# serviceberry3/weiner_slamit_v2

Hardware: AMD Instinct MI355X
Metric: frames/sec ORB extract+match @640x480x8lvl (higher is better)
Workload: dtype u8; 1 GPU; BASELINE configs[1]: 640x480 8-level ORB extract (1000 features, FAST 20/7) + brute-force 256-bit Hamming best/second match vs the stream's previous frame; 256 independent streams per GPU per step; distinct_frame_pairs_per_gpu=16, parallelism=streams sharded over 1 GPU(s), no data-path collective

## Files before the change

### weiner_slamit_v2_amd/csrc/orb_api.hip

```cpp
#include <hip/hip_runtime.h>
#include <math.h>
#include <stdio.h>
#include <stdlib.h>
#include <string.h>

#include <algorithm>
#include <vector>

#include "../../include/slamit.h"
#include "orb_plan.h"
#include "slamit_internal.h"

hipError_t orbk_upload_pattern(hipStream_t st);
void orbk_resize(hipStream_t st, const uint8_t* src, int sw, int sh, size_t sstride, size_t sframe,
                 uint8_t* dst, int dw, int dh, size_t dstride, size_t dframe, const int* xofs,
                 const short* ialpha, const int* yofs, const short* ibeta, int nframes);
void orbk_resize_rows4(hipStream_t st, const uint8_t* src, size_t sstride, size_t sframe, int sh, uint8_t* dst, int dw, int dh,
                       size_t dstride, size_t dframe, const uint32_t* d_col, const uint32_t* d_row, int nframes);
void orbk_resize_rows8(hipStream_t st, const uint8_t* src, size_t sstride, size_t sframe, int sh, uint8_t* dst, int dw, int dh,
                       size_t dstride, size_t dframe, const uint32_t* d_col8, const uint32_t* d_row, int nframes);
hipError_t orbk_pyramid_bands_prepare(int smem_bytes);
void orbk_pyramid_bands(hipStream_t st, const BandTab& tab, const uint8_t* d_tables, const BandRows* d_rows, int first, int last, int nbands,
                        const uint8_t* src, size_t sstride, size_t sframe, int sh, uint8_t* pyr, size_t pyr_frame, int tile0, int smem, int nframes);
hipError_t orbk_pyramid_prepare(int smem_bytes);
void orbk_pyramid(hipStream_t st, const OrbLevel* levels, int nlevels, const PyrBox* boxes, const PyrTabs* tabs,
                  int nregions, const uint8_t* img0, size_t img0_stride, size_t img0_frame, uint8_t* pyr, int bufA_bytes,
                  int smem_bytes, int nframes, int l_first, int l_last);
hipError_t orbk_fast_prepare(int max_wcell, int max_hcell);
void orbk_fast(hipStream_t st, const FastTab& tab, int nlevels, const uint32_t* d_cells, int cells_per_frame, const uint8_t* img0,
               size_t img0_stride, size_t img0_frame, const uint8_t* pyr, unsigned long long* cand,
               size_t cand_frame_stride, int* cand_count, int iniTh, int minTh, int max_wcell, int max_hcell, int nframes);
hipError_t orbk_octree_prepare(int node_cap, int key_cap);
void orbk_octree(hipStream_t st, const OrbLevel* levels, int nlevels, const unsigned long long* cand,
                 size_t cand_frame_stride, int* cand_count, uint32_t* ws_xy, uint16_t* ws_node,
                 OrbLevelKp* lkp, size_t kp_frame_stride, int* kp_count, int node_cap, int key_cap, int nframes,
                 int level_override);
void orbk_ic_angle(hipStream_t st, const OrbLevel* levels, int nlevels, const uint8_t* img0, size_t img0_stride,
                   size_t img0_frame, const uint8_t* pyr, OrbLevelKp* lkp, size_t kp_frame_stride,
                   const int* kp_count, int max_kp, int nframes);
void orbk_blur_stream(hipStream_t st, const OrbLevel* levels, const uint32_t* d_tiles, int ntiles, const uint8_t* img0,
                      size_t img0_stride, size_t img0_frame, const uint8_t* pyr, uint8_t* blur, int nframes, bool edge);
void orbk_blur(hipStream_t st, const OrbLevel* levels, const uint32_t* d_tiles, int total_tiles, const uint8_t* img0,
               size_t img0_stride, size_t img0_frame, const uint8_t* pyr, uint8_t* blur, int nframes);
void orbk_describe(hipStream_t st, const OrbLevel* levels, int nlevels, const uint8_t* blur,
                   const OrbLevelKp* lkp, size_t kp_frame_stride, const int* kp_count, slamit_kp* out_kps,
                   uint8_t* out_desc, int out_cap, int* out_n, int max_kp, int nframes);
void orbk_pad(hipStream_t st, const uint8_t* src, int w, int h, size_t sstride, uint8_t* dst);
void orbk_decode_candidates(hipStream_t st, const OrbLevel* levels, int level, const unsigned long long* K, int n,
                            unsigned long long* order_out, int* xys);

namespace {

inline size_t round_up(size_t v, size_t a) { return (v + a - 1) / a * a; }

}

#define ORB_BLUR_SPLIT 1

struct slamit_orb {
    slamit_orb_params p;
    int device;
    hipStream_t stream;
    hipStream_t stream_b;
    hipEvent_t ev_pyr, ev_mid, ev_blur;
    SlamitSwitches sw;
    int nlevels;
    OrbPlan pl;
    bool blur_stream_on;
    uint8_t* d_tables;
    const OrbLevel* d_levels;
    uint8_t* d_pyr;
    uint8_t* d_blur;
    unsigned long long* d_cand;
    uint32_t* d_ws_xy;
    uint16_t* d_ws_node;
    int* d_counts;
    bool counters_clean;
    OrbLevelKp* d_lkp;
    uint8_t* d_in;
    size_t d_in_stride, d_in_frame;
    slamit_kp* d_out_kps;
    uint8_t* d_out_desc;
    int* d_out_n;
    uint8_t* h_out;
    uint8_t* d_scratch;
    size_t scratch_bytes;
    int prof_on;
    long prof_call;
    std::vector<hipEvent_t> prof_ev;
    std::vector<int> prof_stage;
    const uint8_t* last_img0;
    size_t last_stride, last_frame;
    int last_nframes;
};

template <typename T>
static const T* dtab(const slamit_orb* h, size_t off) { return reinterpret_cast<const T*>(h->d_tables + off); }

static void orb_free(slamit_orb* h) {
    if (!h) return;
    SlamitDeviceGuard guard(h->device);
    hipFree(h->d_tables); hipFree(h->d_pyr); hipFree(h->d_blur); hipFree(h->d_cand); hipFree(h->d_ws_xy);
    hipFree(h->d_ws_node); hipFree(h->d_counts); hipFree(h->d_lkp); hipFree(h->d_in); hipFree(h->d_out_kps);
    hipFree(h->d_out_desc); hipFree(h->d_out_n); if (h->h_out) hipHostFree(h->h_out); hipFree(h->d_scratch);
    for (hipEvent_t e : h->prof_ev) hipEventDestroy(e);
    if (h->ev_pyr) hipEventDestroy(h->ev_pyr);
    if (h->ev_mid) hipEventDestroy(h->ev_mid);
    if (h->ev_blur) hipEventDestroy(h->ev_blur);
    if (h->stream_b) hipStreamDestroy(h->stream_b);
    if (h->stream) hipStreamDestroy(h->stream);
    delete h;
}

extern "C" {

int slamit_orb_create(const slamit_orb_params* p, int device, slamit_orb** out) {
    if (!p || !out) return slamit_fail(SLAMIT_ERR_ARG, "slamit_orb_create: null argument");
    *out = nullptr;
    if (p->nlevels < 1 || p->nlevels > ORB_MAX_LEVELS || p->nfeatures < 1 || !(p->scale_factor > 1.f) ||
        p->ini_th_fast < 1 || p->ini_th_fast > 255 || p->min_th_fast < 1 || p->min_th_fast > 255 ||
        p->width < 0 || p->height < 0 || p->max_batch < 1)
        return slamit_fail(SLAMIT_ERR_ARG, "slamit_orb_create: parameter out of range");
    SLAMIT_USE_DEVICE(device);
    slamit_orb* h = new slamit_orb();
    h->p = *p;
    h->device = device;
    h->sw = slamit_read_switches();
    const int nl = h->nlevels = p->nlevels;
    const char* why = "";
// ... 118 lines not shown
        }
    };
    prof_mark(h, st, ST_RESIZE, true);
    const bool src0_aligned = ((((uintptr_t)d_gray) | stride | frame_stride) & 3) == 0;
    const bool side = h->prof_on != 1;
    const bool early_blur = side && ORB_BLUR_SPLIT < nl - 1;
    int early_done = -1;
    auto fork_early_blur = [&](int l) -> hipError_t {
        hipError_t e = hipEventRecord(h->ev_mid, st);
        if (e == hipSuccess) e = hipStreamWaitEvent(h->stream_b, h->ev_mid, 0);
        if (e != hipSuccess) return e;
        launch_blur(h->stream_b, 0, l + 1);
        early_done = l;
        return hipSuccess;
    };
    if (!P.bands.empty() && src0_aligned) {
        for (const OrbBandSeg& G : P.bands) {
            const OrbLevel& S = P.levels[G.first];
            orbk_pyramid_bands(st, P.band_tab, h->d_tables, dtab<BandRows>(h, G.rows_off), G.first, G.last, G.nbands,
                               G.first == 0 ? d_gray : h->d_pyr + S.plane_off, G.first == 0 ? stride : (size_t)S.stride,
                               G.first == 0 ? frame_stride : P.pyr_frame_total, S.h, h->d_pyr, P.pyr_frame_total, G.tile0, G.smem, nframes);
            if (early_blur && G.last < nl - 1 && early_done < 0) HIP_TRY(fork_early_blur(G.last));
        }
    } else if (P.rows4_ok && src0_aligned) {
        for (int l = 1; l < nl; ++l) {
            const OrbLevel& S = P.levels[l - 1];
            const OrbLevel& D = P.levels[l];
            const uint8_t* src = l == 1 ? d_gray : h->d_pyr + S.plane_off;
            const OrbResizeTabs& T = P.rs[l];
            if (!T.col8.empty())
                orbk_resize_rows8(st, src, l == 1 ? stride : (size_t)S.stride, l == 1 ? frame_stride : P.pyr_frame_total, S.h,
                                  h->d_pyr + D.plane_off, D.w, D.h, (size_t)D.stride, P.pyr_frame_total, dtab<uint32_t>(h, T.col8_off),
                                  dtab<uint32_t>(h, T.row4_off), nframes);
            else
                orbk_resize_rows4(st, src, l == 1 ? stride : (size_t)S.stride, l == 1 ? frame_stride : P.pyr_frame_total, S.h,
                                  h->d_pyr + D.plane_off, D.w, D.h, (size_t)D.stride, P.pyr_frame_total, dtab<uint32_t>(h, T.col4_off),
                                  dtab<uint32_t>(h, T.row4_off), nframes);
            if (early_blur && l == ORB_BLUR_SPLIT) HIP_TRY(fork_early_blur(l));
        }
    } else if (P.pyr_regions) {
        orbk_pyramid(st, h->d_levels, nl, dtab<PyrBox>(h, P.boxes_off), dtab<PyrTabs>(h, P.tabs_off), P.pyr_regions, d_gray, stride, frame_stride,
                     h->d_pyr, P.pyr_bufA, P.pyr_smem, nframes, 0, nl - 1);
    } else {
        for (int l = 1; l < nl; ++l) {
            const OrbLevel& S = P.levels[l - 1];
            const OrbLevel& D = P.levels[l];
            const uint8_t* src = l == 1 ? d_gray : h->d_pyr + S.plane_off;
            size_t sstride = l == 1 ? stride : (size_t)S.stride;
            size_t sframe = l == 1 ? frame_stride : P.pyr_frame_total;
            const OrbResizeTabs& T = P.rs[l];
            orbk_resize(st, src, S.w, S.h, sstride, sframe, h->d_pyr + D.plane_off, D.w, D.h, (size_t)D.stride,
                        P.pyr_frame_total, dtab<int>(h, T.xofs_off), dtab<short>(h, T.ialpha_off), dtab<int>(h, T.yofs_off),
                        dtab<short>(h, T.ibeta_off), nframes);
        }
    }
    prof_mark(h, st, ST_RESIZE, false);
    prof_mark(h, st, ST_FAST, true);
    orbk_fast(st, P.fast, nl, dtab<uint32_t>(h, P.cells_off), (int)(P.cells.size() / 4), d_gray, stride, frame_stride, h->d_pyr, h->d_cand,
              P.cand_frame_stride, cand_count, h->p.ini_th_fast, h->p.min_th_fast, P.max_wcell, P.max_hcell, nframes);
    prof_mark(h, st, ST_FAST, false);
    if (side) {
        HIP_TRY(hipEventRecord(h->ev_pyr, st));
        HIP_TRY(hipStreamWaitEvent(h->stream_b, h->ev_pyr, 0));
        launch_blur(h->stream_b, early_done + 1, nl);
        HIP_TRY(hipEventRecord(h->ev_blur, h->stream_b));
    }
    prof_mark(h, st, ST_OCTREE, true);
    orbk_octree(st, h->d_levels, nl, h->d_cand, P.cand_frame_stride, cand_count, h->d_ws_xy, h->d_ws_node, h->d_lkp,
                P.kp_frame_stride, kp_count, P.node_cap, P.oct_key_cap, nframes, -1);
    prof_mark(h, st, ST_OCTREE, false);
    prof_mark(h, st, ST_ANGLE, true);
    orbk_ic_angle(st, h->d_levels, nl, d_gray, stride, frame_stride, h->d_pyr, h->d_lkp, P.kp_frame_stride, kp_count,
                  P.max_kp_level, nframes);
    prof_mark(h, st, ST_ANGLE, false);
    if (side) {
        HIP_TRY(hipStreamWaitEvent(st, h->ev_blur, 0));
    } else {
        prof_mark(h, st, ST_BLUR, true);
        launch_blur(st, 0, nl);
        prof_mark(h, st, ST_BLUR, false);
    }
    prof_mark(h, st, ST_DESCRIBE, true);
    orbk_describe(st, h->d_levels, nl, h->d_blur, h->d_lkp, P.kp_frame_stride, kp_count, d_kps, d_desc, cap, d_n_out,
                  P.max_kp_level, nframes);
    prof_mark(h, st, ST_DESCRIBE, false);
    ++h->prof_call;
    HIP_TRY(hipGetLastError());
    h->counters_clean = true;
    h->last_img0 = d_gray; h->last_stride = stride; h->last_frame = frame_stride; h->last_nframes = nframes;
    return SLAMIT_OK;
}

int slamit_orb_extract_batch(slamit_orb* h, const uint8_t* gray, size_t stride, size_t frame_stride, int nframes,
                             slamit_kp* kps, uint8_t* desc, int cap, int* n_out) {
    if (!h || !n_out || nframes < 0) return slamit_fail(SLAMIT_ERR_ARG, "slamit_orb_extract_batch: bad argument");
    if (nframes > h->p.max_batch) return slamit_fail(SLAMIT_ERR_CAPACITY, "slamit_orb_extract_batch: nframes > max_batch");
    if (nframes == 0) return SLAMIT_OK;
    if (h->p.width == 0 || h->p.height == 0) {
        for (int f = 0; f < nframes; ++f) n_out[f] = 0;
        return SLAMIT_OK;
    }
    if (!gray || !kps || !desc) return slamit_fail(SLAMIT_ERR_ARG, "slamit_orb_extract_batch: null buffer");
    if (cap < h->pl.max_out) return slamit_fail(SLAMIT_ERR_CAPACITY, "slamit_orb_extract_batch: cap < slamit_orb_max_keypoints()");
    SLAMIT_USE_DEVICE(h->device);
    const int W = h->p.width, H = h->p.height;
    for (int f = 0; f < nframes; ++f)
        HIP_TRY(hipMemcpy2DAsync(h->d_in + f * h->d_in_frame, h->d_in_stride, gray + (size_t)f * frame_stride, stride, W, H,
                                 hipMemcpyHostToDevice, h->stream));
    int rc = slamit_orb_extract_batch_dev(h, h->d_in, h->d_in_stride, h->d_in_frame, nframes, h->d_out_kps, h->d_out_desc,
                                          h->pl.max_out, h->d_out_n, h->stream);
    if (rc != SLAMIT_OK) return rc;
    const size_t o_k = ((sizeof(int) * (size_t)nframes + 255) & ~(size_t)255), kb = sizeof(slamit_kp) * (size_t)h->pl.max_out * nframes;
    const size_t o_d = (o_k + kb + 255) & ~(size_t)255, db = (size_t)SLAMIT_DESC_BYTES * h->pl.max_out * nframes;
    HIP_TRY(hipMemcpyAsync(h->h_out, h->d_out_n, sizeof(int) * nframes, hipMemcpyDeviceToHost, h->stream));
    HIP_TRY(hipMemcpyAsync(h->h_out + o_k, h->d_out_kps, kb, hipMemcpyDeviceToHost, h->stream));
    HIP_TRY(hipMemcpyAsync(h->h_out + o_d, h->d_out_desc, db, hipMemcpyDeviceToHost, h->stream));
    HIP_TRY(hipStreamSynchronize(h->stream));
    memcpy(n_out, h->h_out, sizeof(int) * nframes);
    for (int f = 0; f < nframes; ++f) {
        const int n = n_out[f];
        if (n > 0) {
            memcpy(kps + (size_t)f * cap, h->h_out + o_k + sizeof(slamit_kp) * (size_t)f * h->pl.max_out, sizeof(slamit_kp) * n);
            memcpy(desc + (size_t)f * cap * SLAMIT_DESC_BYTES, h->h_out + o_d + (size_t)SLAMIT_DESC_BYTES * f * h->pl.max_out, (size_t)SLAMIT_DESC_BYTES * n);
        }
    }
    return SLAMIT_OK;
}

int slamit_orb_extract(slamit_orb* h, const uint8_t* gray, size_t stride, slamit_kp* kps, uint8_t* desc, int cap,
                       int* n_out) {
    return slamit_orb_extract_batch(h, gray, stride, stride * (size_t)(h ? h->p.height : 0), 1, kps, desc, cap, n_out);
}

int slamit_orb_profile(slamit_orb* h, int enable, float* stage_ms, int32_t* stage_calls, int nstages) {
    if (!h) return slamit_fail(SLAMIT_ERR_ARG, "slamit_orb_profile: null handle");
    SLAMIT_USE_DEVICE(h->device);
    if (stage_ms || stage_calls) {
        for (int i = 0; i < nstages; ++i) { if (stage_ms) stage_ms[i] = 0.f; if (stage_calls) stage_calls[i] = 0; }
        for (size_t i = 0; i < h->prof_stage.size() && 2 * i + 1 < h->prof_ev.size(); ++i) {
            HIP_TRY(hipEventSynchronize(h->prof_ev[2 * i + 1]));
            float ms = 0.f;
            HIP_TRY(hipEventElapsedTime(&ms, h->prof_ev[2 * i], h->prof_ev[2 * i + 1]));
            int s = h->prof_stage[i];
            if (s < nstages) { if (stage_ms) stage_ms[s] += ms; if (stage_calls) stage_calls[s] += 1; }
        }
    }
    for (hipEvent_t e : h->prof_ev) hipEventDestroy(e);
    h->prof_ev.clear(); h->prof_stage.clear();
    h->prof_on = enable;
    h->prof_call = 0;
    return SLAMIT_OK;
}

int slamit_orb_level(slamit_orb* h, int frame, int level, uint8_t* dst, size_t dst_bytes, int* w, int* h_out) {
    if (!h || level < 0 || level >= h->nlevels) return slamit_fail(SLAMIT_ERR_ARG, "slamit_orb_level: bad level");
    if (h->p.width == 0 || h->p.height == 0) return slamit_fail(SLAMIT_ERR_STATE, "slamit_orb_level: empty image");
    const OrbLevel& L = h->pl.levels[level];
    if (w) *w = L.w;
    if (h_out) *h_out = L.h;
    if (!dst) return SLAMIT_OK;
    if (frame < 0 || frame >= h->last_nframes || !h->last_img0) return slamit_fail(SLAMIT_ERR_STATE, "slamit_orb_level: no such frame in the last extract call");
    size_t need = (size_t)(L.w + 38) * (L.h + 38);
    if (dst_bytes < need) return slamit_fail(SLAMIT_ERR_CAPACITY, "slamit_orb_level: dst too small");
    SLAMIT_USE_DEVICE(h->device);
    const uint8_t* src = level == 0 ? h->last_img0 + (size_t)frame * h->last_frame
                                    : h->d_pyr + L.plane_off + (size_t)frame * h->pl.pyr_frame_total;
    orbk_pad(h->stream, src, L.w, L.h, level == 0 ? h->last_stride : (size_t)L.stride, h->d_scratch);
// ... 68 lines not shown
```

### weiner_slamit_v2_amd/csrc/orb_kernels.hip

```cpp
#include <hip/hip_runtime.h>
#include <stdint.h>

#include <algorithm>

#include "orb_types.h"
#include "slamit_math.h"
#include "wave_ops.h"
#include "../../include/slamit.h"
#include "../../include/slamit_orb_pattern.h"

#define WAVE 64

__global__ __launch_bounds__(256) void resize_level_kernel(
    const uint8_t* __restrict__ src, int sw, int sh, size_t sstride, size_t sframe,
    uint8_t* __restrict__ dst, int dw, int dh, size_t dstride, size_t dframe,
    const int* __restrict__ xofs, const short* __restrict__ ialpha,
    const int* __restrict__ yofs, const short* __restrict__ ibeta) {
    const int x4 = (blockIdx.x * 64 + (threadIdx.x & 63)) * 4;
    const int y = blockIdx.y * 4 + (threadIdx.x >> 6);
    const int f = blockIdx.z;
    if (x4 >= dw || y >= dh) return;
    const uint8_t* S = src + (size_t)f * sframe;
    int sy = yofs[y];
    int sy0 = min(max(sy, 0), sh - 1), sy1 = min(max(sy + 1, 0), sh - 1);
    const uint8_t* S0 = S + (size_t)sy0 * sstride;
    const uint8_t* S1 = S + (size_t)sy1 * sstride;
    int b0 = ibeta[2 * y], b1 = ibeta[2 * y + 1];
    uint32_t out = 0;
#pragma unroll
    for (int i = 0; i < 4; ++i) {
        int x = x4 + i;
        if (x < dw) {
            int sx = xofs[x];
            int sx1 = min(sx + 1, sw - 1);
            int a0 = ialpha[2 * x], a1 = ialpha[2 * x + 1];
            int r0 = S0[sx] * a0 + S0[sx1] * a1;
            int r1 = S1[sx] * a0 + S1[sx1] * a1;
            int v = ((((b0 * (r0 >> 4)) >> 16) + ((b1 * (r1 >> 4)) >> 16) + 2) >> 2) & 0xFF;
            out |= (uint32_t)v << (8 * i);
        }
    }
    *reinterpret_cast<uint32_t*>(dst + (size_t)f * dframe + (size_t)y * dstride + x4) = out;
}

typedef unsigned short rs_us2 __attribute__((ext_vector_type(2)));
typedef unsigned rs_u3 __attribute__((ext_vector_type(3)));
__device__ __forceinline__ uint32_t rs_dot2(uint32_t taps, uint32_t alpha) {
    return __builtin_amdgcn_udot2(__builtin_bit_cast(rs_us2, taps), __builtin_bit_cast(rs_us2, alpha), 0u, false);
}

#define RS_RP 2

template <int RP>
__device__ __forceinline__ void rs_item(const int item, const uint8_t* S, const unsigned ss, const unsigned sbytes, uint8_t* D, const unsigned dstride,
                                        const uint4* __restrict__ coltab, const uint2* __restrict__ rowtab, const int ngroups,
                                        const unsigned inv_groups, const int dh) {
    const int yq = (int)__umulhi((unsigned)item, inv_groups);
    const int g = item - yq * ngroups;
    const uint8_t* ct = reinterpret_cast<const uint8_t*>(coltab) + 48u * (unsigned)g;
    const uint4 c0 = *reinterpret_cast<const uint4*>(ct), c1 = *reinterpret_cast<const uint4*>(ct + 16u);
    const uint32_t c2x = *reinterpret_cast<const uint32_t*>(ct + 32u);
    int yrow[2 * RP];
    uint2 rt[2 * RP];
    {
        const uint4* rp4 = reinterpret_cast<const uint4*>(reinterpret_cast<const uint8_t*>(rowtab) + 16u * (unsigned)(RP * yq));
#pragma unroll
        for (int r = 0; r < RP; ++r) {
            const uint4 v = rp4[r];
            rt[2 * r] = make_uint2(v.x, v.y); rt[2 * r + 1] = make_uint2(v.z, v.w);
        }
#pragma unroll
        for (int r = 0; r < 2 * RP; ++r) yrow[r] = min(2 * RP * yq + r, dh - 1);
    }
    const unsigned b = c0.x & 0xFFFFu, sh = (c0.x >> 16) & 3u, off1 = (c0.x >> 20) & 15u, off2 = (c0.x >> 24) & 15u;
    const uint32_t sel[4] = {c0.y, c0.z, c0.w, c1.x}, al[4] = {c1.y, c1.z, c1.w, c2x};
    uint32_t w[4 * RP][3];
    const __amdgpu_buffer_rsrc_t rsrc = __builtin_amdgcn_make_buffer_rsrc(const_cast<uint8_t*>(S), 0, sbytes, 0x00020000);
    (void)off1; (void)off2;
#pragma unroll
    for (int r = 0; r < 4 * RP; ++r) {
        const unsigned srow = (r & 1) ? (rt[r >> 1].x >> 16) : (rt[r >> 1].x & 0xFFFFu);
        const unsigned ro = __umul24(srow, ss) + b;
        const rs_u3 v = __builtin_amdgcn_raw_buffer_load_b96(rsrc, (int)ro, 0, 0);
        w[r][0] = v.x; w[r][1] = v.y; w[r][2] = v.z;
    }
#pragma unroll
    for (int k = 0; k < 2 * RP; ++k) {
// ... 1419 lines not shown
    };
    auto rotate = [&]() {
        const blur_u3 ta = qa[0], tb = qb[0];
        qa[0] = qa[1]; qb[0] = qb[1]; qa[1] = qa[2]; qb[1] = qb[2]; qa[2] = ta; qb[2] = tb;
#pragma unroll
        for (int j = 0; j < 4; ++j) { P[0][j] = P[1][j]; P[1][j] = P[2][j]; P[2][j] = P[3][j]; }
    };
#define BLUR_OUT(f, k0, k1, k2, k3, j) \
    min((udot2(P[(f) & 3][j], k3, udot2(P[((f) + 3) & 3][j], k2, udot2(P[((f) + 2) & 3][j], k1, udot2(P[((f) + 1) & 3][j], k0, 1u << 15)))) >> 16), 255u)
#define BLUR_OUT_A(f) (BLUR_OUT(f, kA0, kA1, kA2, kA3, 0) | (BLUR_OUT(f, kA0, kA1, kA2, kA3, 1) << 8) | (BLUR_OUT(f, kA0, kA1, kA2, kA3, 2) << 16) | (BLUR_OUT(f, kA0, kA1, kA2, kA3, 3) << 24))
#define BLUR_OUT_B(f) (BLUR_OUT(f, kB0, kB1, kB2, kB3, 0) | (BLUR_OUT(f, kB0, kB1, kB2, kB3, 1) << 8) | (BLUR_OUT(f, kB0, kB1, kB2, kB3, 2) << 16) | (BLUR_OUT(f, kB0, kB1, kB2, kB3, 3) << 24))
    auto generic = [&](const int p) {
        const blur_u3 na = fetch(2 * p + 6), nb = fetch(2 * p + 7);
        advance(0, 3, na, nb);
        const int ya = 2 * p - 3, yb = 2 * p - 2;
        if (ya >= by0 && ya <= ylast) *reinterpret_cast<uint32_t*>(D + __umul24((unsigned)ya, ds)) = BLUR_OUT_A(3);
        if (yb >= by0 && yb <= ylast) *reinterpret_cast<uint32_t*>(D + __umul24((unsigned)yb, ds)) = BLUR_OUT_B(3);
        rotate();
    };
    int p = p0;
#pragma unroll
    for (int k = 0; k < 3; ++k, ++p) advance(k, k, fetch(2 * p + 6), fetch(2 * p + 7));
    generic(p);
    ++p;
    const int n = min((ylast + 2) >> 1, (h - 8) >> 1) - p + 1;
    int nu = 0;
    {
        const unsigned long long act = __ballot(1);
#pragma unroll
        for (int b = 32; b; b >>= 1) nu += __ballot(n >= nu + b) == act ? b : 0;
    }
    if (nu > 0) {
        const uint8_t* sp = S + __umul24((unsigned)(2 * p + 6), ss);
        uint8_t* dp = D + __umul24((unsigned)(2 * p - 3), ds);
        p += nu;
        auto steady = [&](const int q, const int f) {
            const blur_u3 na = fetch_row(sp);
            sp += ss;
            const blur_u3 nb = fetch_row(sp);
            sp += ss;
            advance(q, f, na, nb);
            *reinterpret_cast<uint32_t*>(dp) = BLUR_OUT_A(f);
            dp += ds;
            *reinterpret_cast<uint32_t*>(dp) = BLUR_OUT_B(f);
            dp += ds;
            asm volatile("" : "+v"(sp), "+v"(dp));
        };
        for (; nu >= 12; nu -= 12) {
#pragma unroll
            for (int u = 0; u < 12; ++u) {
                steady(u % 3, (u + 3) & 3);
                __builtin_amdgcn_sched_barrier(0);
            }
        }
        for (; nu >= 3; nu -= 3) {
#pragma unroll
            for (int u = 0; u < 3; ++u) {
                steady(u, (u + 3) & 3);
                __builtin_amdgcn_sched_barrier(0);
            }
#pragma unroll
            for (int j = 0; j < 4; ++j) { P[2][j] = P[1][j]; P[1][j] = P[0][j]; P[0][j] = P[3][j]; }
        }
#pragma unroll 1
        for (; nu > 0; --nu) {
            steady(0, 3);
            rotate();
        }
    }
#pragma unroll 4
    for (; p <= p1; ++p) generic(p);
#undef BLUR_OUT_B
#undef BLUR_OUT_A
#undef BLUR_OUT
}

__constant__ __attribute__((aligned(16))) signed char c_pattern[SLAMIT_ORB_PATTERN_INTS];
#define DESC_KP_PER_WAVE 4
#define DESC_R 18
#define DESC_ROWS (2 * DESC_R + 1)
#define DESC_PITCH 48
#define DESC_LOADS 2

__global__ __launch_bounds__(256) void describe_kernel(
    const OrbLevel* __restrict__ levels, int nlevels,
    const uint8_t* __restrict__ blur,
    const OrbLevelKp* __restrict__ lkp, size_t kp_frame_stride, const int* __restrict__ kp_count,
    slamit_kp* __restrict__ out_kps, uint8_t* __restrict__ out_desc, int out_cap,
    int* __restrict__ out_n, int xcd_frames , int kblocks) {
    const int lane = threadIdx.x & 63;
    int level, frame, kb;
    if (xcd_frames) {
        const unsigned w = blockIdx.x, k = w >> 3, P = (unsigned)(nlevels * kblocks), fq = k / P, local = k - fq * P;
        frame = (int)(8u * fq + ((w + fq) & 7u));
        if (frame >= xcd_frames) return;
        level = (int)(local / (unsigned)kblocks); kb = (int)(local - (unsigned)level * (unsigned)kblocks);
    } else { level = blockIdx.y; frame = blockIdx.z; kb = blockIdx.x; }
    const int i0 = (kb * 4 + (threadIdx.x >> 6)) * DESC_KP_PER_WAVE;
    const OrbLevel& L = levels[level];
    const int* counts = kp_count + frame * nlevels;
    int offset = 0, total = 0;
    for (int l = 0; l < nlevels; ++l) {
        int c = counts[l];
        if (l < level) offset += c;
        total += c;
    }
    if (level == 0 && i0 == 0 && lane == 0) out_n[frame] = min(total, out_cap);
    const int count = counts[level];
    if (i0 >= count) return;
    const int4 pw = reinterpret_cast<const int4*>(c_pattern)[lane];
    const int pt[4] = {pw.x, pw.y, pw.z, pw.w};
    float px0[4], py0[4], px1[4], py1[4];
#pragma unroll
    for (int t = 0; t < 4; ++t) {
        px0[t] = (float)(signed char)(pt[t] & 0xFF); py0[t] = (float)(signed char)((pt[t] >> 8) & 0xFF);
        px1[t] = (float)(signed char)((pt[t] >> 16) & 0xFF); py1[t] = (float)(signed char)((pt[t] >> 24) & 0xFF);
    }
    const uint8_t* img = blur + L.blur_off + (size_t)frame * L.blur_bytes;
    const unsigned step = (unsigned)L.stride;
    const OrbLevelKp* KP = lkp + L.kp_off + (size_t)frame * kp_frame_stride;
    OrbLevelKp kp[DESC_KP_PER_WAVE];
#pragma unroll
    for (int k = 0; k < DESC_KP_PER_WAVE; ++k) kp[k] = KP[min(i0 + k, count - 1)];
    __shared__ __attribute__((aligned(16))) uint8_t s_patch[4][DESC_KP_PER_WAVE][DESC_ROWS * DESC_PITCH];
    const int wv = threadIdx.x >> 6;
    int lrow[DESC_LOADS], lcol[DESC_LOADS];
    unsigned poff[DESC_LOADS];
#pragma unroll
    for (int it = 0; it < DESC_LOADS; ++it) {
        const int idx = lane + 64 * it;
        lrow[it] = (int)(((unsigned)idx * 21846u) >> 16);
        lcol[it] = idx - 3 * lrow[it];
        poff[it] = __umul24((unsigned)min(lrow[it], DESC_ROWS - 1), step) + 16u * (unsigned)lcol[it];
    }
    const __amdgpu_buffer_rsrc_t rsrc = __builtin_amdgcn_make_buffer_rsrc(const_cast<uint8_t*>(img), 0, (unsigned)L.stride * (unsigned)L.h, 0x00020000);
    typedef unsigned desc_u4 __attribute__((ext_vector_type(4)));
    desc_u4 ld[DESC_KP_PER_WAVE][DESC_LOADS];
#pragma unroll
    for (int k = 0; k < DESC_KP_PER_WAVE; ++k) {
        const unsigned base = __umul24((unsigned)(kp[k].y - DESC_R), step) + (unsigned)((kp[k].x - DESC_R) & ~3);
#pragma unroll
        for (int it = 0; it < DESC_LOADS; ++it) ld[k][it] = __builtin_amdgcn_raw_buffer_load_b128(rsrc, (int)(base + poff[it]), 0, 0);
    }
#pragma unroll
    for (int k = 0; k < DESC_KP_PER_WAVE; ++k)
#pragma unroll
        for (int it = 0; it < DESC_LOADS; ++it)
            if (lrow[it] < DESC_ROWS) *reinterpret_cast<desc_u4*>(&s_patch[wv][k][__mul24(lrow[it], DESC_PITCH) + 16 * lcol[it]]) = ld[k][it];
    __builtin_amdgcn_fence(__ATOMIC_ACQ_REL, "wavefront");
    __builtin_amdgcn_wave_barrier();
    typedef float desc_f2 __attribute__((ext_vector_type(2)));
    const desc_f2 magic = {12582912.0f, 12582912.0f};
    const unsigned DESC_BIAS = 0x400000u * (unsigned)DESC_PITCH + 0x4B400000u;
    int tv0[DESC_KP_PER_WAVE][4], tv1[DESC_KP_PER_WAVE][4];
#pragma unroll
    for (int k = 0; k < DESC_KP_PER_WAVE; ++k) {
        const float a = kp[k].cs, b = kp[k].sn;
        const desc_f2 ba = {b, a}, anb = {a, -b};
        const uint8_t* center = &s_patch[wv][k][DESC_R * DESC_PITCH + DESC_R + ((kp[k].x - DESC_R) & 3)];
        const uint8_t* biased = center - DESC_BIAS;
#pragma unroll
        for (int t = 0; t < 4; ++t) {
            const desc_f2 p0 = {px0[t], px0[t]}, q0 = {py0[t], py0[t]}, p1 = {px1[t], px1[t]}, q1 = {py1[t], py1[t]};
            const desc_f2 m0 = (p0 * ba + q0 * anb) + magic, m1 = (p1 * ba + q1 * anb) + magic;
            tv0[k][t] = biased[__umul24(__float_as_uint(m0.x), (unsigned)DESC_PITCH) + __float_as_uint(m0.y)];
            tv1[k][t] = biased[__umul24(__float_as_uint(m1.x), (unsigned)DESC_PITCH) + __float_as_uint(m1.y)];
        }
    }
#pragma unroll
    for (int k = 0; k < DESC_KP_PER_WAVE; ++k) {
        const int i = i0 + k, o = offset + i;
        unsigned nib = 0;
#pragma unroll
        for (int t = 0; t < 4; ++t) nib |= (unsigned)(tv0[k][t] < tv1[k][t]) << t;
        unsigned other = __shfl_xor(nib, 1, WAVE);
        if (i >= count || o >= out_cap) continue;
        if ((lane & 1) == 0)
            out_desc[((size_t)frame * out_cap + o) * SLAMIT_DESC_BYTES + (lane >> 1)] = (uint8_t)(nib | (other << 4));
        if (lane == 0) {
            slamit_kp kk;
            float fx = (float)kp[k].x, fy = (float)kp[k].y;
            if (level != 0) { fx *= L.scale; fy *= L.scale; }
            kk.x = fx; kk.y = fy; kk.size = L.patch_size; kk.angle = kp[k].angle; kk.response = kp[k].response;
            kk.octave = level; kk.class_id = -1;
            out_kps[(size_t)frame * out_cap + o] = kk;
        }
    }
}

__global__ __launch_bounds__(256) void pad_level_kernel(const uint8_t* __restrict__ src, int w, int h,
                                                        size_t sstride, uint8_t* __restrict__ dst) {
    const int B = SLAMIT_EDGE_THRESHOLD;
    const int pw = w + 2 * B, ph = h + 2 * B;
    int x = blockIdx.x * 64 + (threadIdx.x & 63), y = blockIdx.y * 4 + (threadIdx.x >> 6);
    if (x >= pw || y >= ph) return;
    dst[(size_t)y * pw + x] = src[(size_t)reflect101(y - B, h) * sstride + reflect101(x - B, w)];
}

__global__ void decode_candidates_kernel(const OrbLevel* __restrict__ levels, int level,
                                         const unsigned long long* __restrict__ K, int n,
                                         unsigned long long* __restrict__ order_out, int* __restrict__ xys) {
    int k = blockIdx.x * blockDim.x + threadIdx.x;
    if (k >= n) return;
    const OrbLevel& L = levels[level];
    unsigned long long c = K[k];
    unsigned order = (unsigned)c;
    int lx = order & 63, ly = (order >> 6) & 63, cell = order >> 12;
    int ci = cell / L.nCols, cj = cell - ci * L.nCols;
    xys[3 * k + 0] = cj * L.wCell + lx;
    xys[3 * k + 1] = ci * L.hCell + ly;
    xys[3 * k + 2] = (int)(c >> 32);
    order_out[k] = order;
}

extern "C++" {

hipError_t orbk_upload_pattern(hipStream_t st) {
    static const DiscTable disc = make_disc();
    hipError_t e = hipMemcpyToSymbolAsync(HIP_SYMBOL(c_disc), &disc, sizeof(disc), 0, hipMemcpyHostToDevice, st);
    if (e != hipSuccess) return e;
    return hipMemcpyToSymbolAsync(HIP_SYMBOL(c_pattern), slamit_orb_pattern, SLAMIT_ORB_PATTERN_INTS, 0,
                                  hipMemcpyHostToDevice, st);
}

void orbk_resize(hipStream_t st, const uint8_t* src, int sw, int sh, size_t sstride, size_t sframe,
                 uint8_t* dst, int dw, int dh, size_t dstride, size_t dframe, const int* xofs,
                 const short* ialpha, const int* yofs, const short* ibeta, int nframes) {
    dim3 grid((dw + 255) / 256, (dh + 3) / 4, nframes);
    hipLaunchKernelGGL(resize_level_kernel, grid, dim3(256), 0, st, src, sw, sh, sstride, sframe, dst, dw,
                       dh, dstride, dframe, xofs, ialpha, yofs, ibeta);
}

hipError_t orbk_pyramid_prepare(int smem_bytes) {
    return hipFuncSetAttribute(reinterpret_cast<const void*>(pyramid_fused_kernel),
                               hipFuncAttributeMaxDynamicSharedMemorySize, smem_bytes);
}

void orbk_pyramid(hipStream_t st, const OrbLevel* levels, int nlevels, const PyrBox* boxes, const PyrTabs* tabs,
                  int nregions, const uint8_t* img0, size_t img0_stride, size_t img0_frame, uint8_t* pyr, int bufA_bytes,
                  int smem_bytes, int nframes, int l_first, int l_last) {
    hipLaunchKernelGGL(pyramid_fused_kernel, dim3(nregions, nframes), dim3(PYR_THREADS), smem_bytes, st, levels, nlevels, boxes,
                       tabs, img0, img0_stride, img0_frame, pyr, bufA_bytes, l_first, l_last);
}

#ifndef FAST_PS
#define FAST_PS 48
#define FAST_PL 80
#endif
static int fast_pitch(int max_wcell) { return max_wcell + 11 <= FAST_PS ? FAST_PS : FAST_PL; }

size_t orbk_fast_smem(int max_wcell, int max_hcell) {
    const int P = fast_pitch(max_wcell);
    const int tile_rows = max_hcell + 6, sc_rows = max_hcell + 2;
    const int kp_cap = ((max_wcell + 1) / 2) * ((max_hcell + 1) / 2);
    return (size_t)4 * fast_wave_bytes(P, tile_rows, sc_rows, kp_cap);
}

hipError_t orbk_fast_prepare(int max_wcell, int max_hcell) {
    const int smem = (int)orbk_fast_smem(max_wcell, max_hcell);
    hipError_t e;
    if (fast_pitch(max_wcell) == FAST_PS) {
        e = hipFuncSetAttribute(reinterpret_cast<const void*>(fast_cells_kernel<FAST_PS>), hipFuncAttributeMaxDynamicSharedMemorySize, smem);
    } else {
        e = hipFuncSetAttribute(reinterpret_cast<const void*>(fast_cells_kernel<FAST_PL>), hipFuncAttributeMaxDynamicSharedMemorySize, smem);
    }
    return e;
}

void orbk_fast(hipStream_t st, const FastTab& tab, int nlevels, const uint32_t* d_cells, int cells_per_frame,
               const uint8_t* img0, size_t img0_stride, size_t img0_frame, const uint8_t* pyr,
               unsigned long long* cand, size_t cand_frame_stride, int* cand_count, int iniTh, int minTh,
               int max_wcell, int max_hcell, int nframes) {
// ... 1 lines not shown
    const int kp_cap = ((max_wcell + 1) / 2) * ((max_hcell + 1) / 2);
    const int wpb = cells_per_frame < 1600 ? 1 : 4;
    const int xcd_frames = nframes >= 16 ? nframes : 0;
    const dim3 grid = xcd_frames ? dim3((unsigned)(((nframes + 7) / 8) * 8) * (unsigned)((cells_per_frame + wpb - 1) / wpb))
                                 : dim3(wpb == 1 ? (unsigned)((cells_per_frame + 31) & ~31) : (unsigned)((cells_per_frame + wpb - 1) / wpb), nframes);
    const size_t smem = orbk_fast_smem(max_wcell, max_hcell) / 4 * wpb;
    if (fast_pitch(max_wcell) == FAST_PS)
        hipLaunchKernelGGL(fast_cells_kernel<FAST_PS>, grid, dim3(64 * wpb), smem, st, tab, reinterpret_cast<const uint4*>(d_cells), nlevels, cells_per_frame, img0,
                           (unsigned)img0_stride, img0_frame, pyr, cand, cand_frame_stride, cand_count, iniTh, minTh, tile_rows,
                           sc_rows, kp_cap, xcd_frames);
    else
        hipLaunchKernelGGL(fast_cells_kernel<FAST_PL>, grid, dim3(64 * wpb), smem, st, tab, reinterpret_cast<const uint4*>(d_cells), nlevels, cells_per_frame, img0,
                           (unsigned)img0_stride, img0_frame, pyr, cand, cand_frame_stride, cand_count, iniTh, minTh, tile_rows,
                           sc_rows, kp_cap, xcd_frames);
}

hipError_t orbk_octree_prepare(int node_cap, int key_cap) {
    static int prepared = 0;
    const int want = (int)orbk_octree_smem(node_cap, key_cap);
    if (want <= prepared) return hipSuccess;
    prepared = want;
    hipError_t e = hipFuncSetAttribute(reinterpret_cast<const void*>(octree_kernel<256>), hipFuncAttributeMaxDynamicSharedMemorySize, want);
    if (e != hipSuccess) return e;
    e = hipFuncSetAttribute(reinterpret_cast<const void*>(octree_kernel<OCT_THREADS>), hipFuncAttributeMaxDynamicSharedMemorySize, want);
    if (e != hipSuccess) return e;
    return hipFuncSetAttribute(reinterpret_cast<const void*>(octree_kernel<1024>), hipFuncAttributeMaxDynamicSharedMemorySize, want);
}

void orbk_octree(hipStream_t st, const OrbLevel* levels, int nlevels, const unsigned long long* cand,
                 size_t cand_frame_stride, int* cand_count, uint32_t* ws_xy, uint16_t* ws_node,
                 OrbLevelKp* lkp, size_t kp_frame_stride, int* kp_count, int node_cap, int key_cap, int nframes,
                 int level_override) {
    dim3 grid(nframes, level_override >= 0 ? 1 : nlevels);
    const int nt = nframes >= 96 ? 256 : nframes <= 16 ? 1024 : OCT_THREADS;
    if (nframes >= 96) key_cap = std::min(key_cap, 2048);
    if (nt == 1024)
        hipLaunchKernelGGL(octree_kernel<1024>, grid, dim3(1024), orbk_octree_smem(node_cap, key_cap), st, levels, nlevels, cand,
                           cand_frame_stride, cand_count, ws_xy, ws_node, lkp, kp_frame_stride, kp_count, node_cap,
                           key_cap, level_override);
    else if (nt == 256)
        hipLaunchKernelGGL(octree_kernel<256>, grid, dim3(256), orbk_octree_smem(node_cap, key_cap), st, levels, nlevels, cand,
                           cand_frame_stride, cand_count, ws_xy, ws_node, lkp, kp_frame_stride, kp_count, node_cap,
                           key_cap, level_override);
    else
        hipLaunchKernelGGL(octree_kernel<OCT_THREADS>, grid, dim3(OCT_THREADS), orbk_octree_smem(node_cap, key_cap), st, levels, nlevels, cand,
                           cand_frame_stride, cand_count, ws_xy, ws_node, lkp, kp_frame_stride, kp_count, node_cap,
                           key_cap, level_override);
}

void orbk_ic_angle(hipStream_t st, const OrbLevel* levels, int nlevels, const uint8_t* img0,
                   size_t img0_stride, size_t img0_frame, const uint8_t* pyr, OrbLevelKp* lkp,
                   size_t kp_frame_stride, const int* kp_count, int max_kp, int nframes) {
    const int kblocks = (max_kp + 4 * IC_KP_PER_WAVE - 1) / (4 * IC_KP_PER_WAVE);
    if (nframes >= 16)
        hipLaunchKernelGGL(ic_angle_kernel, dim3((unsigned)(((nframes + 7) / 8) * 8 * nlevels * kblocks)), dim3(256), 0, st, levels,
                           nlevels, img0, img0_stride, img0_frame, pyr, lkp, kp_frame_stride, kp_count, nframes, kblocks);
    else
        hipLaunchKernelGGL(ic_angle_kernel, dim3(kblocks, nlevels, nframes), dim3(256), 0, st, levels,
                           nlevels, img0, img0_stride, img0_frame, pyr, lkp, kp_frame_stride, kp_count, 0, kblocks);
}

void orbk_blur_stream(hipStream_t st, const OrbLevel* levels, const uint32_t* d_tiles, int ntiles, const uint8_t* img0,
                      size_t img0_stride, size_t img0_frame, const uint8_t* pyr, uint8_t* blur, int nframes, bool edge) {
    if (ntiles <= 0) return;
    if (edge)
        hipLaunchKernelGGL(blur_stream_kernel<true>, dim3((ntiles + 15) / 16, nframes), dim3(256), 0, st, levels, reinterpret_cast<const uint4*>(d_tiles), img0,
                           img0_stride, img0_frame, pyr, blur, (unsigned)ntiles);
    else
        hipLaunchKernelGGL(blur_stream_kernel<false>, dim3((ntiles + 15) / 16, nframes), dim3(256), 0, st, levels, reinterpret_cast<const uint4*>(d_tiles), img0,
                           img0_stride, img0_frame, pyr, blur, (unsigned)ntiles);
}

void orbk_blur(hipStream_t st, const OrbLevel* levels, const uint32_t* d_tiles, int total_tiles, const uint8_t* img0,
               size_t img0_stride, size_t img0_frame, const uint8_t* pyr, uint8_t* blur, int nframes) {
    if (total_tiles <= 0) return;
    const unsigned total = (unsigned)total_tiles * (unsigned)nframes, grid = ((total + 7u) >> 3) << 3;
    const unsigned inv = (unsigned)((0x100000000ull + (unsigned)total_tiles - 1) / (unsigned)total_tiles);
    hipLaunchKernelGGL(blur_all_kernel, dim3(grid), dim3(256), 0, st, levels, reinterpret_cast<const uint4*>(d_tiles), img0,
                       img0_stride, img0_frame, pyr, blur, (unsigned)total_tiles, inv, total);
}

void orbk_describe(hipStream_t st, const OrbLevel* levels, int nlevels, const uint8_t* blur,
                   const OrbLevelKp* lkp, size_t kp_frame_stride, const int* kp_count, slamit_kp* out_kps,
                   uint8_t* out_desc, int out_cap, int* out_n, int max_kp, int nframes) {
    const int kblocks = (max_kp + 4 * DESC_KP_PER_WAVE - 1) / (4 * DESC_KP_PER_WAVE);
    if (nframes >= 16)
        hipLaunchKernelGGL(describe_kernel, dim3((unsigned)(((nframes + 7) / 8) * 8 * nlevels * kblocks)), dim3(256), 0, st, levels,
                           nlevels, blur, lkp, kp_frame_stride, kp_count, out_kps, out_desc, out_cap, out_n, nframes, kblocks);
    else
        hipLaunchKernelGGL(describe_kernel, dim3(kblocks, nlevels, nframes), dim3(256), 0, st, levels,
                           nlevels, blur, lkp, kp_frame_stride, kp_count, out_kps, out_desc, out_cap, out_n, 0, kblocks);
}

void orbk_pad(hipStream_t st, const uint8_t* src, int w, int h, size_t sstride, uint8_t* dst) {
    hipLaunchKernelGGL(pad_level_kernel, dim3((w + 38 + 63) / 64, (h + 38 + 3) / 4), dim3(256), 0, st, src, w, h,
                       sstride, dst);
}

void orbk_decode_candidates(hipStream_t st, const OrbLevel* levels, int level, const unsigned long long* K,
                            int n, unsigned long long* order_out, int* xys) {
    if (n <= 0) return;
    hipLaunchKernelGGL(decode_candidates_kernel, dim3((n + 255) / 256), dim3(256), 0, st, levels, level, K, n,
                       order_out, xys);
}

}
```

Before: 320,100 frames/s.

## Add level-walking describe kernel sized to expected keypoints with software-pipelined fetch

For batches of 16 or more frames, describe now launches a new kernel. Its grid is sized from the expected feature count rather than nlevels × max_kp blocks per frame. Each wave walks a cursor across pyramid levels, taking groups of four keypoints spaced by a global stride. It prefetches the next group's patch loads through buffer loads while computing taps for the current group, which removes the many empty blocks of the old per-level grid and hides load latency. The cost is serial per-wave work, extra register pressure, and dependence on the nfeatures estimate for load balance.

Result: no change. 323,100 frames/s, median of 6 (+0.9%).

```diff
diff --git a/weiner_slamit_v2_amd/csrc/orb_api.hip b/weiner_slamit_v2_amd/csrc/orb_api.hip
--- a/weiner_slamit_v2_amd/csrc/orb_api.hip
+++ b/weiner_slamit_v2_amd/csrc/orb_api.hip
@@ -44,7 +44,7 @@
                size_t img0_stride, size_t img0_frame, const uint8_t* pyr, uint8_t* blur, int nframes);
 void orbk_describe(hipStream_t st, const OrbLevel* levels, int nlevels, const uint8_t* blur,
                    const OrbLevelKp* lkp, size_t kp_frame_stride, const int* kp_count, slamit_kp* out_kps,
-                   uint8_t* out_desc, int out_cap, int* out_n, int max_kp, int nframes);
+                   uint8_t* out_desc, int out_cap, int* out_n, int max_kp, int expect_kp, int nframes);
 void orbk_pad(hipStream_t st, const uint8_t* src, int w, int h, size_t sstride, uint8_t* dst);
 void orbk_decode_candidates(hipStream_t st, const OrbLevel* levels, int level, const unsigned long long* K, int n,
                             unsigned long long* order_out, int* xys);
@@ -329,7 +329,7 @@
     }
     prof_mark(h, st, ST_DESCRIBE, true);
     orbk_describe(st, h->d_levels, nl, h->d_blur, h->d_lkp, P.kp_frame_stride, kp_count, d_kps, d_desc, cap, d_n_out,
-                  P.max_kp_level, nframes);
+                  P.max_kp_level, h->p.nfeatures, nframes);
     prof_mark(h, st, ST_DESCRIBE, false);
     ++h->prof_call;
     HIP_TRY(hipGetLastError());
diff --git a/weiner_slamit_v2_amd/csrc/orb_gather.h b/weiner_slamit_v2_amd/csrc/orb_gather.h
--- /dev/null
+++ b/weiner_slamit_v2_amd/csrc/orb_gather.h
@@ -0,0 +1,48 @@
+#ifndef SLAMIT_ORB_GATHER_H
+#define SLAMIT_ORB_GATHER_H
+
+#ifdef __HIPCC__
+#define ORB_GATHER_HD __host__ __device__
+#else
+#define ORB_GATHER_HD
+#endif
+
+#define ORB_GATHER_WAVES 4
+
+struct OrbGatherCursor {
+    int level;
+    int first;
+    int before;
+    int count;
+};
+
+ORB_GATHER_HD inline int orb_gather_groups(int count, int G) { return (count + G - 1) / G; }
+
+ORB_GATHER_HD inline int orb_gather_first(int slice, int wave) { return slice * ORB_GATHER_WAVES + wave; }
+ORB_GATHER_HD inline int orb_gather_step(int slices) { return slices * ORB_GATHER_WAVES; }
+
+template <class Counts>
+ORB_GATHER_HD inline void orb_gather_begin(OrbGatherCursor& c, const Counts& counts, int nlevels) {
+    c.level = 0; c.first = 0; c.before = 0;
+    c.count = nlevels > 0 ? counts(0) : 0;
+}
+
+template <class Counts>
+ORB_GATHER_HD inline bool orb_gather_seek(OrbGatherCursor& c, const Counts& counts, int nlevels, int G, int g, int* i0) {
+    while (c.level < nlevels) {
+        const int n = orb_gather_groups(c.count, G);
+        if (g < c.first + n) { *i0 = (g - c.first) * G; return true; }
+        c.first += n; c.before += c.count; ++c.level;
+        c.count = c.level < nlevels ? counts(c.level) : 0;
+    }
+    return false;
+}
+
+ORB_GATHER_HD inline int orb_gather_slices(int expect_kp, int G, int per_wave, int cap) {
+    const int per_slice = ORB_GATHER_WAVES * per_wave;
+    int s = (orb_gather_groups(expect_kp, G) + per_slice - 1) / per_slice;
+    if (s > cap) s = cap;
+    return s < 1 ? 1 : s;
+}
+
+#endif
diff --git a/weiner_slamit_v2_amd/csrc/orb_kernels.hip b/weiner_slamit_v2_amd/csrc/orb_kernels.hip
--- a/weiner_slamit_v2_amd/csrc/orb_kernels.hip
+++ b/weiner_slamit_v2_amd/csrc/orb_kernels.hip
@@ -3,6 +3,7 @@
 
 #include <algorithm>
 
+#include "orb_gather.h"
 #include "orb_types.h"
 #include "slamit_math.h"
 #include "wave_ops.h"
@@ -1588,6 +1589,97 @@
 #define DESC_PITCH 48
 #define DESC_LOADS 2
 
+typedef unsigned desc_u4 __attribute__((ext_vector_type(4)));
+struct DescLane {
+    float px0[4], py0[4], px1[4], py1[4];
+    int lrow[DESC_LOADS], lcol[DESC_LOADS];
+};
+
+__device__ __forceinline__ void desc_lane_setup(DescLane& W, int lane) {
+    const int4 pw = reinterpret_cast<const int4*>(c_pattern)[lane];
+    const int pt[4] = {pw.x, pw.y, pw.z, pw.w};
+#pragma unroll
+    for (int t = 0; t < 4; ++t) {
+        W.px0[t] = (float)(signed char)(pt[t] & 0xFF); W.py0[t] = (float)(signed char)((pt[t] >> 8) & 0xFF);
+        W.px1[t] = (float)(signed char)((pt[t] >> 16) & 0xFF); W.py1[t] = (float)(signed char)((pt[t] >> 24) & 0xFF);
+    }
+#pragma unroll
+    for (int it = 0; it < DESC_LOADS; ++it) {
+        const int idx = lane + 64 * it;
+        W.lrow[it] = (int)(((unsigned)idx * 21846u) >> 16);
+        W.lcol[it] = idx - 3 * W.lrow[it];
+    }
+}
+
+__device__ __forceinline__ void desc_chunk_offsets(unsigned (&poff)[DESC_LOADS], const DescLane& W, unsigned step) {
+#pragma unroll
+    for (int it = 0; it < DESC_LOADS; ++it) poff[it] = __umul24((unsigned)min(W.lrow[it], DESC_ROWS - 1), step) + 16u * (unsigned)W.lcol[it];
+}
+
+__device__ __forceinline__ void desc_fetch(desc_u4 (&ld)[DESC_KP_PER_WAVE][DESC_LOADS], __amdgpu_buffer_rsrc_t rsrc, unsigned step,
+                                           const unsigned (&poff)[DESC_LOADS], const OrbLevelKp (&kp)[DESC_KP_PER_WAVE]) {
+#pragma unroll
+    for (int k = 0; k < DESC_KP_PER_WAVE; ++k) {
+        const unsigned base = __umul24((unsigned)(kp[k].y - DESC_R), step) + (unsigned)((kp[k].x - DESC_R) & ~3);
+#pragma unroll
+        for (int it = 0; it < DESC_LOADS; ++it) ld[k][it] = __builtin_amdgcn_raw_buffer_load_b128(rsrc, (int)(base + poff[it]), 0, 0);
+    }
+}
+
+__device__ __forceinline__ void desc_stage(uint8_t (*patch)[DESC_ROWS * DESC_PITCH], const DescLane& W,
+                                           const desc_u4 (&ld)[DESC_KP_PER_WAVE][DESC_LOADS]) {
+#pragma unroll
+    for (int k = 0; k < DESC_KP_PER_WAVE; ++k)
+#pragma unroll
+        for (int it = 0; it < DESC_LOADS; ++it)
+            if (W.lrow[it] < DESC_ROWS) *reinterpret_cast<desc_u4*>(&patch[k][__mul24(W.lrow[it], DESC_PITCH) + 16 * W.lcol[it]]) = ld[k][it];
+    __builtin_amdgcn_fence(__ATOMIC_ACQ_REL, "wavefront");
+    __builtin_amdgcn_wave_barrier();
+}
+
+__device__ __forceinline__ void desc_taps_store(const uint8_t (*patch)[DESC_ROWS * DESC_PITCH], const DescLane& W,
+                                                const OrbLevelKp (&kp)[DESC_KP_PER_WAVE], int i0, int count, int offset, int level,
+                                                float scale, float patch_size, int frame, slamit_kp* __restrict__ out_kps,
+                                                uint8_t* __restrict__ out_desc, int out_cap, int lane) {
+    typedef float desc_f2 __attribute__((ext_vector_type(2)));
+    const desc_f2 magic = {12582912.0f, 12582912.0f};
+    const unsigned DESC_BIAS = 0x400000u * (unsigned)DESC_PITCH + 0x4B400000u;
+    int tv0[DESC_KP_PER_WAVE][4], tv1[DESC_KP_PER_WAVE][4];
+#pragma unroll
+    for (int k = 0; k < DESC_KP_PER_WAVE; ++k) {
+        const float a = kp[k].cs, b = kp[k].sn;
+        const desc_f2 ba = {b, a}, anb = {a, -b};
+        const uint8_t* center = &patch[k][DESC_R * DESC_PITCH + DESC_R + ((kp[k].x - DESC_R) & 3)];
+        const uint8_t* biased = center - DESC_BIAS;
+#pragma unroll
+        for (int t = 0; t < 4; ++t) {
+            const desc_f2 p0 = {W.px0[t], W.px0[t]}, q0 = {W.py0[t], W.py0[t]}, p1 = {W.px1[t], W.px1[t]}, q1 = {W.py1[t], W.py1[t]};
+            const desc_f2 m0 = (p0 * ba + q0 * anb) + magic, m1 = (p1 * ba + q1 * anb) + magic;
+            tv0[k][t] = biased[__umul24(__float_as_uint(m0.x), (unsigned)DESC_PITCH) + __float_as_uint(m0.y)];
+            tv1[k][t] = biased[__umul24(__float_as_uint(m1.x), (unsigned)DESC_PITCH) + __float_as_uint(m1.y)];
+        }
+    }
+#pragma unroll
+    for (int k = 0; k < DESC_KP_PER_WAVE; ++k) {
+        const int i = i0 + k, o = offset + i;
+        unsigned nib = 0;
+#pragma unroll
+        for (int t = 0; t < 4; ++t) nib |= (unsigned)(tv0[k][t] < tv1[k][t]) << t;
+        unsigned other = __shfl_xor(nib, 1, WAVE);
+        if (i >= count || o >= out_cap) continue;
+        if ((lane & 1) == 0)
+            out_desc[((size_t)frame * out_cap + o) * SLAMIT_DESC_BYTES + (lane >> 1)] = (uint8_t)(nib | (other << 4));
+        if (lane == 0) {
+            slamit_kp kk;
+            float fx = (float)kp[k].x, fy = (float)kp[k].y;
+            if (level != 0) { fx *= scale; fy *= scale; }
+            kk.x = fx; kk.y = fy; kk.size = patch_size; kk.angle = kp[k].angle; kk.response = kp[k].response;
+            kk.octave = level; kk.class_id = -1;
+            out_kps[(size_t)frame * out_cap + o] = kk;
+        }
+    }
+}
+
 __global__ __launch_bounds__(256) void describe_kernel(
     const OrbLevel* __restrict__ levels, int nlevels,
     const uint8_t* __restrict__ blur,
@@ -1694,6 +1786,94 @@
     }
 }
 
+#define DESC_WALK_MIN_FRAMES 16
+#define DESC_GROUPS_PER_WAVE 2
+
+struct GatherCounts {
+    int mine;
+    __device__ __forceinline__ void load(const int* __restrict__ counts, int nlevels, int lane) { mine = lane < nlevels ? counts[lane] : 0; }
+    __device__ __forceinline__ int operator()(int level) const { return __builtin_amdgcn_readlane(mine, level); }
+    __device__ __forceinline__ int total() const {
+        int t = 0;
+#pragma unroll
+        for (int l = 0; l < ORB_MAX_LEVELS; ++l) t += __builtin_amdgcn_readlane(mine, l);
+        return t;
+    }
+};
+
+__device__ __forceinline__ OrbLevelKp uniform_kp(const OrbLevelKp& r) {
+    OrbLevelKp u;
+    const int xy = __builtin_amdgcn_readfirstlane((int)(uint16_t)r.x | ((int)r.y << 16));
+    u.x = (int16_t)(xy & 0xFFFF); u.y = (int16_t)(xy >> 16);
+    u.response = __int_as_float(__builtin_amdgcn_readfirstlane(__float_as_int(r.response)));
+    u.angle = __int_as_float(__builtin_amdgcn_readfirstlane(__float_as_int(r.angle)));
+    u.cs = __int_as_float(__builtin_amdgcn_readfirstlane(__float_as_int(r.cs)));
+    u.sn = __int_as_float(__builtin_amdgcn_readfirstlane(__float_as_int(r.sn)));
+    return u;
+}
+
+__global__ __launch_bounds__(256, 5) void describe_walk_kernel(
+    const OrbLevel* __restrict__ levels, int nlevels,
+    const uint8_t* __restrict__ blur,
+    const OrbLevelKp* __restrict__ lkp, size_t kp_frame_stride, const int* __restrict__ kp_count,
+    slamit_kp* __restrict__ out_kps, uint8_t* __restrict__ out_desc, int out_cap,
+    int* __restrict__ out_n, int nframes, int slices) {
+    const int lane = threadIdx.x & 63;
+    const int wv = __builtin_amdgcn_readfirstlane((int)(threadIdx.x >> 6));
+    const unsigned w = blockIdx.x, k = w >> 3, fq = k / (unsigned)slices;
+    const int frame = (int)(8u * fq + ((w + fq) & 7u));
+    const int slice = (int)(k - fq * (unsigned)slices);
+    if (frame >= nframes) return;
+    GatherCounts counts;
+    counts.load(kp_count + frame * nlevels, nlevels, lane);
+    if (slice == 0 && wv == 0 && lane == 0) out_n[frame] = min(counts.total(), out_cap);
+    OrbGatherCursor cur;
+    orb_gather_begin(cur, counts, nlevels);
+    int g = orb_gather_first(slice, wv), i0;
+    if (!orb_gather_seek(cur, counts, nlevels, DESC_KP_PER_WAVE, g, &i0)) return;
+    DescLane W;
+    desc_lane_setup(W, lane);
+    __shared__ __attribute__((aligned(16))) uint8_t s_patch[4][DESC_KP_PER_WAVE][DESC_ROWS * DESC_PITCH];
+    desc_u4 ld[DESC_KP_PER_WAVE][DESC_LOADS];
+    OrbLevelKp kp[DESC_KP_PER_WAVE];
+    int level = -1;
+    unsigned step = 0, plane_bytes = 0, poff[DESC_LOADS] = {0, 0};
+    float scale = 0.f, patch_size = 0.f;
+    const uint8_t* img = nullptr;
+    const OrbLevelKp* KP = nullptr;
+    auto fetch = [&](int first) {
+        if (cur.level != level) {
+            level = cur.level;
+            const OrbLevel& L = levels[level];
+            img = blur + L.blur_off + (size_t)frame * L.blur_bytes;
+            step = (unsigned)L.stride; plane_bytes = (unsigned)L.stride * (unsigned)L.h;
+            scale = L.scale; patch_size = L.patch_size;
+            KP = lkp + L.kp_off + (size_t)frame * kp_frame_stride;
+            desc_chunk_offsets(poff, W, step);
+        }
+#pragma unroll
+        for (int k = 0; k < DESC_KP_PER_WAVE; ++k) kp[k] = uniform_kp(KP[min(first + k, cur.count - 1)]);
+        desc_fetch(ld, __builtin_amdgcn_make_buffer_rsrc(const_cast<uint8_t*>(img), 0, (unsigned)__builtin_amdgcn_readfirstlane((int)plane_bytes), 0x00020000),
+                   step, poff, kp);
+    };
+    fetch(i0);
+    int i_now, count_now, offset_now, level_now;
+    float scale_now, patch_now;
+    for (;;) {
+        desc_stage(s_patch[wv], W, ld);
+        i_now = i0; count_now = cur.count; offset_now = cur.before; level_now = level; scale_now = scale; patch_now = patch_size;
+        g += orb_gather_step(slices);
+        if (!orb_gather_seek(cur, counts, nlevels, DESC_KP_PER_WAVE, g, &i0)) break;
+        desc_taps_store(s_patch[wv], W, kp, i_now, count_now, offset_now, level_now, scale_now, patch_now, frame, out_kps, out_desc,
+                        out_cap, lane);
+        __builtin_amdgcn_sched_barrier(0);
+        fetch(i0);
+        wave_sync_lds();
+    }
+    desc_taps_store(s_patch[wv], W, kp, i_now, count_now, offset_now, level_now, scale_now, patch_now, frame, out_kps, out_desc,
+                    out_cap, lane);
+}
+
 __global__ __launch_bounds__(256) void pad_level_kernel(const uint8_t* __restrict__ src, int w, int h,
                                                         size_t sstride, uint8_t* __restrict__ dst) {
     const int B = SLAMIT_EDGE_THRESHOLD;
@@ -1861,12 +2041,13 @@
 
 void orbk_describe(hipStream_t st, const OrbLevel* levels, int nlevels, const uint8_t* blur,
                    const OrbLevelKp* lkp, size_t kp_frame_stride, const int* kp_count, slamit_kp* out_kps,
-                   uint8_t* out_desc, int out_cap, int* out_n, int max_kp, int nframes) {
+                   uint8_t* out_desc, int out_cap, int* out_n, int max_kp, int expect_kp, int nframes) {
     const int kblocks = (max_kp + 4 * DESC_KP_PER_WAVE - 1) / (4 * DESC_KP_PER_WAVE);
-    if (nframes >= 16)
-        hipLaunchKernelGGL(describe_kernel, dim3((unsigned)(((nframes + 7) / 8) * 8 * nlevels * kblocks)), dim3(256), 0, st, levels,
-                           nlevels, blur, lkp, kp_frame_stride, kp_count, out_kps, out_desc, out_cap, out_n, nframes, kblocks);
-    else
+    if (nframes >= DESC_WALK_MIN_FRAMES) {
+        const int slices = orb_gather_slices(expect_kp, DESC_KP_PER_WAVE, DESC_GROUPS_PER_WAVE, nlevels * kblocks);
+        hipLaunchKernelGGL(describe_walk_kernel, dim3((unsigned)(((nframes + 7) / 8) * 8 * slices)), dim3(256), 0, st, levels,
+                           nlevels, blur, lkp, kp_frame_stride, kp_count, out_kps, out_desc, out_cap, out_n, nframes, slices);
+    } else
         hipLaunchKernelGGL(describe_kernel, dim3(kblocks, nlevels, nframes), dim3(256), 0, st, levels,
                            nlevels, blur, lkp, kp_frame_stride, kp_count, out_kps, out_desc, out_cap, out_n, 0, kblocks);
 }
```
